# henrycharlesworth/settlers_of_catan_RL

Hardware: AMD Instinct MI355X
Metric: Catan env-steps/sec at 65k parallel games (higher is better)
Workload: dtype u8/u32 (integer bitboards); 1 GPU; configs[1]: 65 536 parallel envs per GPU, random policy, step+mask only, bit-exact vs CPU oracle; games_per_gpu=65536, games_total=65536, validate_actions=True, auto_reset=True, parallelism=games sharded over 1 GPU(s), no collective

## Files before the change

### settlers_of_catan_rl_amd/csrc/catan_kernels.hip

```cpp
#include <hip/hip_runtime.h>
#include <stdint.h>

#include "catan_state.h"

#define CATAN_TABLE static __device__ __constant__ const
#define CATAN_FN static __device__ __forceinline__
#define CATAN_TOPOLOGY_CODE
#include "catan_topology.inc"

namespace catan {

#define DEVI __device__ __forceinline__

constexpr int BLOCK = 256;
constexpr u64 ALL54 = (1ull << 54) - 1;

constexpr int MT_RING = 8192, MT_AHEAD = 6144, MT_AHEAD_PY = 1024;
struct MtGen { u32 mt[624]; u32 idx; u32 produced; u32 ring[MT_RING]; };
struct MtPair { MtGen np, py; u32 cons_py; };
struct BoardCfg {
    int32_t randomise;
    int32_t fixed_terrain;
    int32_t fixed_numbers;
    int8_t terrain[19];
// ... 1409 lines not shown
            tmask &= tmask - 1;
            const int r0 = (s.b(B_TILE + t) & 15) - 1;
            const u64 tm = tct[t];
            u32 add = 0;
#pragma unroll
            for (int p = 0; p < 4; p++) add |= (u32)(__popcll(st[p] & tm) + 2 * __popcll(ct[p] & tm)) << (8 * p);
#pragma unroll
            for (int k = 0; k < 5; k++) alloc[k] += (k == r0) ? add : 0u;
        }
    }
    const int res_order[5] = { R_WOOD, R_ORE, R_BRICK, R_WHEAT, R_SHEEP };
    u32 okbits = 0;
#pragma unroll
    for (int i = 0; i < 5; i++) {
        int r0 = res_order[i];
        u32 al = alloc[r0];
        int tot = (al & 255) + ((al >> 8) & 255) + ((al >> 16) & 255) + (al >> 24);
        int bank = s.b(B_BANK + r0);
        if (tot <= bank) { okbits |= 1u << r0; if (tot) s.sb(B_BANK + r0, bank - tot); }
    }
    if (tk) { const long long t1 = clock_fenced(); tk[1] = (u32)(t1 - t0); t0 = t1; }
    u32 mw = 0;
#pragma unroll
    for (int r = 0; r < 4; r++) mw |= ((okbits >> r) & 1) ? 0xFFu << (8 * r) : 0u;
    const u32 mc = ((okbits >> 4) & 1) ? 0xFFFFu : 0u;
    u32 pw[4], tw[4], pc[4], tc[4];
#pragma unroll
    for (int X = 0; X < 4; X++) {
        int hand[5], tot = 0;
#pragma unroll
        for (int r = 0; r < 5; r++) { hand[r] = s.res(X, r); tot += hand[r]; }
        int add[5], bound[5];
#pragma unroll
        for (int r = 0; r < 5; r++) add[r] = ((okbits >> r) & 1) ? (int)((alloc[r] >> (8 * X)) & 255) : 0;
#pragma unroll
        for (int i = 0; i < 5; i++) { const int r = res_order[i]; tot += add[r]; bound[r] = tot; }
#pragma unroll
        for (int r = 0; r < 5; r++) s.spb(X, P_RES + r, hand[r] + add[r]);
        pw[X] = (u32)add[0] | ((u32)add[1] << 8) | ((u32)add[2] << 16) | ((u32)add[3] << 24);
        tw[X] = (u32)bound[0] | ((u32)bound[1] << 8) | ((u32)bound[2] << 16) | ((u32)bound[3] << 24);
        pc[X] = (u32)add[4] * 0x0101u; tc[X] = (u32)bound[4] * 0x0101u;
    }
    int base[12];
    u32 ea[12], eb[12], ec[12], guard = 0;
#pragma unroll
    for (int X = 0; X < 4; X++)
#pragma unroll
        for (int j = 0; j < 3; j++) {
            const int o = j + (j >= X ? 1 : 0), k = X * 3 + j;
            base[k] = W_EST + (o * 3 + label_of(seatof, o, X)) * 3;
            ea[k] = s.w(base[k]); eb[k] = s.w(base[k] + 1); ec[k] = s.w(base[k] + 2);
            guard |= ea[k] | eb[k] | ec[k] | (ea[k] + pw[X]) | (eb[k] + pw[X]) | (ec[k] + pc[X]) | pw[X] | pc[X] | tw[X] | tc[X];
        }
    if ((guard & H4) == 0) {
#pragma unroll
        for (int X = 0; X < 4; X++)
#pragma unroll
            for (int j = 0; j < 3; j++) {
                const int k = X * 3 + j;
                s.sw(base[k], swar_addmin(ea[k], pw[X], tw[X], mw));
                s.sw(base[k] + 1, swar_addmin(eb[k], pw[X], tw[X], mw));
                s.sw(base[k] + 2, swar_addmin(ec[k], pc[X], tc[X], mc));
            }
    } else {
        for (int X = 0; X < 4; X++)
            for (int o = 0; o < 4; o++)
                if (o != X) est_apply(s, o, label_of(seatof, o, X), pw[X], 0u, tw[X], mw, pc[X], 0u, tc[X], mc);
    }
    if (tk) tk[2] = (u32)(clock_fenced() - t0);
    return roll;
}

template <class S>
DEVI void update_largest_army(const S& s) {
    const int order[4] = { 1, 0, 3, 2 };
    int max_count = 0, who = -1;
#pragma unroll
    for (int i = 0; i < 4; i++) {
        int p = order[i], k = s.pb(p, P_ARMY);
        if (k >= 3 && k > max_count) { max_count = k; who = p; }
    }
    if (who < 0) return;
    int la = s.b(B_LA_PLAYER);
    if (la == 0) { s.sb(B_LA_PLAYER, who + 1); s.sb(B_LA_COUNT, max_count); s.spb(who, P_VP, s.pb(who, P_VP) + 2); }
    else if (la == who + 1) s.sb(B_LA_COUNT, max_count);
    else if (max_count > s.b(B_LA_COUNT)) {
        s.spb(la - 1, P_VP, s.pb(la - 1, P_VP) - 2);
        s.sb(B_LA_PLAYER, who + 1); s.sb(B_LA_COUNT, max_count);
        s.spb(who, P_VP, s.pb(who, P_VP) + 2);
    }
}

struct StepCfg { int validate; int dense_reward; double win_reward; double annealing; Limits lim; int auto_reset;
                 double* reward64;
                 unsigned long long* prof;
                 u32* prof_wave;
                 int prof_timeline;
                 int bin_order; };
constexpr int LRF_PROF_ROW = 4128, LRF_PROF_ROWS = 2000;
constexpr int LRH_PROF_ROW = 6128, LRH_PROF_ROWS = 1000;
constexpr long prof_wave_rows(long N) { return (N / 16 + 17 > LRH_PROF_ROW + LRH_PROF_ROWS) ? N / 16 + 17 : LRH_PROF_ROW + LRH_PROF_ROWS; }
constexpr int PROF_PHASES = 8;
constexpr int PROF_TOTAL = 2 * PROF_PHASES + 4;
constexpr int PROF_WORDS = PROF_TOTAL + 42;
DEVI void prof_mark(const StepCfg& cfg, int phase, long long& t_prev) {
    if (cfg.prof_wave != nullptr) {
        const long long t = wall_clock64();
        if ((threadIdx.x & 63) == 0 && !(cfg.prof_timeline && phase == 2))
            cfg.prof_wave[((long)blockIdx.x * (blockDim.x >> 6) + (threadIdx.x >> 6)) * 8 + phase] = (u32)(t - t_prev);
        t_prev = wall_clock64();
        return;
    }
    if (cfg.prof == nullptr) return;
    long long t = wall_clock64();
    if ((threadIdx.x & 63) == 0) {
        unsigned long long dt = (unsigned long long)(t - t_prev);
        atomicAdd(&cfg.prof[phase], dt);
        atomicMax(&cfg.prof[PROF_PHASES + phase], dt);
    }
    t_prev = wall_clock64();
}

struct Pending { u32* ctr; u64* req[3]; u64* heavy[2]; u64* heavy2; u8* type; u8* who; u64* len; u32* arrive; i32* resets[2][3]; u8* busy;
                 u64* spec;
                 i32* lists;
                 int bsel;
                 int bclear;
                 int fa, ftag, sa, stag;
                 int sample;
                 int lrq_clear;
                 int bnext;
                 int brel;
                 u32* bctr;
                 int nsub;
               };
constexpr int CTR_WORDS = 96;
constexpr int BIN_SETS = 4;
DEVI int lrq_ctr(int fl) { return fl < 2 ? 4 + fl : 7; }
constexpr int NBINS = 18, BIN_NOOP = NBINS - 1;
static_assert(16 + BIN_SETS * NBINS <= CTR_WORDS, "the sets of bin counts live in ctr[16 ..]");
constexpr int BCTR_PAD = 32;
constexpr int MAX_SUBS = 16;
DEVI u32* sub_ctr(const Pending& pend, int set, int bin, int sub) { return pend.bctr + (((long)set * NBINS + bin) * pend.nsub + sub) * BCTR_PAD; }
DEVI i32* sub_list(const Pending& pend, int set, int bin, int sub, long N) { return pend.lists + (((long)set * NBINS + bin) * pend.nsub + sub) * N; }
DEVI int bin_of(int t, int card) {
    if (t < 0 || t > 12) return BIN_NOOP;
    if (t != T_PLAYDEV) return t;
    card = min(max(card, 0), 4);
    return card >= 1 ? 12 + card : t;
}
__device__ constexpr int BIN_ORDER_LPT[18] = { 0, 9, 7, 11, 16, 2, 14, 3, 5, 4, 13, 1, 12, 8, 15, 6, 10, 17 };
DEVI int type_of_bin(int bin) { return bin <= 12 ? bin : (bin < BIN_NOOP ? T_PLAYDEV : -1); }

template <class S>
DEVI void sample_enqueue_lane(const Ctx& c, const S& s, const u32 (&m)[MASK_WORDS], const Pending& pend, u32* __restrict__ mpk) {
    const long e = s.e;
    u32* row = mpk + e * MPK_STRIDE;
    int a[ACTION_WORDS];
    const int t = sample_random(c, s, m, row[ROW_CTR], a, (u32*)nullptr, (u8*)nullptr, 0, 0);
    uint4* dst = reinterpret_cast<uint4*>(row + ROW_ACT);
#pragma unroll
    for (int i = 0; i < 4; i++) dst[i] = make_uint4((u32)a[4 * i], (u32)a[4 * i + 1], (u32)a[4 * i + 2], (u32)a[4 * i + 3]);
    *reinterpret_cast<uint2*>(row + ROW_ACT + 16) = make_uint2((u32)a[16], (u32)a[17]);
    if (pend.brel >= 0) {
        const int bin = bin_of(t, a[4]), sub = (int)(e & (pend.nsub - 1));
        const u32 rank = atomicAdd(sub_ctr(pend, pend.brel, bin, sub), 1u);
        sub_list(pend, pend.brel, bin, sub, c.N)[rank] = (i32)e;
    } else {
        const u32 rank = atomicAdd(&pend.ctr[11 + 4 * pend.sa], 1u);
        pend.resets[pend.sa][2][rank] = (i32)e;
    }
}

struct StepCfg;
DEVI void prof_mark(const StepCfg& cfg, int phase, long long& t_prev);
struct StepScratch { LrWave lr; };

template <int LR, class S>
DEVI void finish_step(const Ctx& c, const S& s, StepScratch* scratch, const StepCfg& cfg, int lane, bool doit, int type,
                      int lr_who, int len, float* __restrict__ reward, u8* __restrict__ done, u32* __restrict__ mpk,
                      long long& tprof, u32 nbr_c, u32 nbr_e, const Pending& pend, int rlist, bool clear_busy,
                      u32* m_out = nullptr, bool* m_valid = nullptr, LrCache* lc = nullptr) {
    const long e = s.e;
    if constexpr (LR != 0) {
        bool cut = false;
        int holder = 0, hcount = 0;
        if constexpr (LR == 2) prof_mark(cfg, 2, tprof);
        if (doit && lr_who >= 0) {
            s.spb(lr_who, P_CURLP, len);
            holder = s.b(B_LR_PLAYER); hcount = s.b(B_LR_COUNT);
            if (holder == 0) {
                if (len >= 5) { s.sb(B_LR_PLAYER, lr_who + 1); s.sb(B_LR_COUNT, len); s.spb(lr_who, P_VP, s.pb(lr_who, P_VP) + 2); }
            } else if (holder == lr_who + 1) {
                if (hcount > len) cut = true; else s.sb(B_LR_COUNT, len);
            } else if (len > hcount) {
                s.spb(holder - 1, P_VP, s.pb(holder - 1, P_VP) - 2);
                s.spb(lr_who, P_VP, s.pb(lr_who, P_VP) + 2);
                s.sb(B_LR_PLAYER, lr_who + 1); s.sb(B_LR_COUNT, len);
            }
        }
        if constexpr (LR == 2) prof_mark(cfg, 5, tprof);
        if constexpr (LR == 2) {
        if (__ballot(cut)) {
            int max_len = len, player = lr_who;
            bool tied = false;
            for (int o = 0; o < 4; o++) {
                const bool mine = cut && o != lr_who;
                const bool need = mine && !lc->valid(o);
                const u64 found = coop_longest_path_packed(need, s, o, scratch->lr, 0, nbr_c, nbr_e);
                if (need) lc->set(o, found & LR_VMASK);
                if (mine) {
                    const int pl = lr_len(lc->get(o));
                    if (pl == max_len) tied = true;
                    else if (pl > max_len) { max_len = pl; tied = false; player = o; }
                }
            }
            if (cut) {
                if (max_len >= 5) {
                    if (tied) {
                        if (player == lr_who) s.sb(B_LR_COUNT, len);
                        else { s.sb(B_LR_PLAYER, 0); s.sb(B_LR_COUNT, 0); s.spb(lr_who, P_VP, s.pb(lr_who, P_VP) - 2); }
                    } else {
                        s.sb(B_LR_PLAYER, player + 1); s.sb(B_LR_COUNT, max_len);
                        s.spb(player, P_VP, s.pb(player, P_VP) + 2);
                        s.spb(lr_who, P_VP, s.pb(lr_who, P_VP) - 2);
                    }
                } else { s.sb(B_LR_PLAYER, 0); s.sb(B_LR_COUNT, 0); s.spb(lr_who, P_VP, s.pb(lr_who, P_VP) - 2); }
            }
        }
        }
    }
    if constexpr (LR == 2) prof_mark(cfg, 3, tprof);
    bool want_reset = false;
    if (doit) {
        const int dict_order[4] = { 1, 3, 2, 0 };
        int vps[4];
#pragma unroll
        for (int p = 0; p < 4; p++) vps[p] = s.pb(p, P_VP);
        int winner = 0;
#pragma unroll
        for (int i = 0; i < 4; i++) if (vps[dict_order[i]] >= 10) winner = dict_order[i] + 1;
        bool dn = winner != 0 && type >= 0;
        double rw[4];
#pragma unroll
        for (int p = 0; p < 4; p++) {
            double r = 0.0;
            if (type >= 0) {
                if (cfg.dense_reward) {
                    r += (double)(5 * (vps[p] - s.b(B_CURVP + p)));
                    if (type == T_PLAYDEV) r += 5.0;
                    if (type == T_ROBBER) r += 1.0;
                    if (type == T_DISCARD) r -= 0.3;
                    if (type == T_CITY) r += 2.5;
                    r *= cfg.annealing;
                }
                s.sb(B_CURVP + p, vps[p]);
                if (dn && winner == p + 1) r += cfg.win_reward;
            }
            rw[p] = r;
        }
        *reinterpret_cast<float4*>(reward + s.e * 4) = make_float4((float)rw[0], (float)rw[1], (float)rw[2], (float)rw[3]);
        if (cfg.reward64) {
            *reinterpret_cast<double2*>(cfg.reward64 + s.e * 4) = make_double2(rw[0], rw[1]);
            *reinterpret_cast<double2*>(cfg.reward64 + s.e * 4 + 2) = make_double2(rw[2], rw[3]);
        }
        if (dn) s.sb(B_WINNER, winner);
        done[s.e] = dn ? 1 : 0;
        want_reset = dn && cfg.auto_reset;
        if (want_reset) pend.resets[pend.sa][rlist][atomicAdd(&pend.ctr[9 + 4 * pend.sa + rlist], 1u)] = (i32)s.e;
        if (want_reset) pend.busy[s.e] = (u8)pend.stag;
        else if (lr_who >= 0 && clear_busy) pend.busy[s.e] = 0;
    }
    if constexpr (LR == 2) prof_mark(cfg, 4, tprof);
    if (doit && !want_reset) {
        u32 m[MASK_WORDS];
        compute_masks(s, m, cfg.lim);
        if (m_out != nullptr) {
#pragma unroll
            for (int i = 0; i < MASK_WORDS; i++) m_out[i] = m[i];
            *m_valid = true;
        } else {
#pragma unroll
            for (int i = 0; i < MASK_WORDS; i++) mpk[e * MPK_STRIDE + i] = m[i];
        }
    }
    prof_mark(cfg, 6, tprof);
}

template <int G, bool SAMPLE = false>
__global__ __launch_bounds__(64) void k_step(Ctx c, const i32* __restrict__ actions, u32* __restrict__ mpk,
                                             float* __restrict__ reward, u8* __restrict__ done,
                                             u32* __restrict__ err, StepCfg cfg, Pending pend, const u32* __restrict__ bins) {
    constexpr int TSG = G + 1;
    typedef StLT<TSG> StG;
    __shared__ u32 tile_all[1][ROWS_HOT * TSG];
    __shared__ u64 tct_all[1][20];
    const int lane = threadIdx.x & 63, wib = threadIdx.x >> 6;
    const int wv = (int)blockIdx.x + wib;
    u32* const tile = tile_all[wib];
    u64* const tct = tct_all[wib];
    if constexpr (SAMPLE) {
        if (wv == 0)
            for (int i = lane; i < NBINS * pend.nsub; i += 64) pend.bctr[((long)pend.bclear * NBINS * pend.nsub + i) * BCTR_PAD] = 0;
        if (wv == 0 && lane == 0 && pend.lrq_clear >= 0) pend.ctr[lrq_ctr(pend.lrq_clear)] = 0;
    } else if (wv == 0 && lane < NBINS) pend.ctr[16 + NBINS * pend.bclear + lane] = 0;
    int bin = -1, cnt = 0, first = 0;
    u32 subc[SAMPLE ? MAX_SUBS : 1];
    if constexpr (SAMPLE) {
        u32 mine[MAX_SUBS], tot = 0;
#pragma unroll
        for (int j = 0; j < MAX_SUBS; j++) mine[j] = (lane < NBINS && j < pend.nsub) ? *sub_ctr(pend, pend.bsel, lane, j) : 0u;
#pragma unroll
        for (int j = 0; j < MAX_SUBS; j++) tot += mine[j];
        const int pos = wv * G;
        int start = 0;
#pragma unroll
        for (int kk = 0; kk < NBINS; kk++) {
            const int k = cfg.bin_order ? BIN_ORDER_LPT[kk] : kk;
            const int ck = __builtin_amdgcn_readlane((int)tot, k), len = (ck + G - 1) & ~(G - 1);
            if (bin < 0 && pos < start + len) { bin = k; cnt = ck; first = pos - start; }
            start += len;
        }
        if (bin < 0) return;
#pragma unroll
        for (int j = 0; j < MAX_SUBS; j++) subc[j] = (u32)__builtin_amdgcn_readlane((int)mine[j], bin);
    } else {
        const int pos = wv * G;
        int start = 0;
#pragma unroll
        for (int kk = 0; kk < NBINS; kk++) {
            const int k = cfg.bin_order ? BIN_ORDER_LPT[kk] : kk;
            const int ck = (int)bins[k], len = (ck + G - 1) & ~(G - 1);
            if (bin < 0 && pos < start + len) { bin = k; cnt = ck; first = pos - start; }
            start += len;
        }
        if (bin < 0) return;
    }
    const int rnk = first + lane;
    long e = 0x7fffffffL;
    if (lane < G && rnk < cnt) {
        if constexpr (SAMPLE) {
            int sub = 0;
            u32 off = (u32)rnk;
#pragma unroll
            for (int j = 0; j < MAX_SUBS - 1; j++) if (sub == j && j + 1 < pend.nsub && off >= subc[j]) { off -= subc[j]; sub = j + 1; }
            e = (long)sub_list(pend, pend.bsel, bin, sub, c.N)[off];
        } else e = (long)pend.lists[((long)pend.bsel * NBINS + bin) * c.N + rnk];
    }
    long long tprof = (cfg.prof || cfg.prof_wave) ? wall_clock64() : 0;
    if (cfg.prof_wave != nullptr && cfg.prof_timeline && lane == 0) cfg.prof_wave[(long)wv * 8 + 2] = (u32)tprof;
    const bool live = e < c.n;
    int type = live ? type_of_bin(bin) : -1;
    if (live && type < 0) {
        *reinterpret_cast<float4*>(reward + e * 4) = make_float4(0.f, 0.f, 0.f, 0.f);
        if (cfg.reward64) { double2* r64 = reinterpret_cast<double2*>(cfg.reward64 + e * 4); r64[0] = make_double2(0.0, 0.0); r64[1] = make_double2(0.0, 0.0); }
        done[e] = 0;
    }
    if (__ballot(type >= 0) == 0) return;
    if (__ballot(type == T_ROLL) != 0 && lane < 19) tct[lane] = topo_tile_corners(lane);
    u32 nbr_c, nbr_e;
    lr_load_nbr(lane, nbr_c, nbr_e);
    int a[ACTION_WORDS];
    const bool t_board = type == T_SETTLE || type == T_ROAD || type == T_CITY;
    const bool t_est = t_board || type == T_BUYDEV || bin == 12 + C_YOP || bin == 12 + C_MONO || type == T_EXCHANGE || type == T_RESPOND ||
                       type == T_ROLL || type == T_STEAL || type == T_DISCARD;
    const bool w_board = __ballot(type >= 0 && t_board) != 0, w_est = __ballot(type >= 0 && t_est) != 0;
    u32 dctr = 0;
    if (w_est) stage_in_all<true, G, SAMPLE>(tile, c.R, actions, type >= 0 ? (int)e : -1, lane, a, mpk, &dctr);
    else stage_in_all<false, G, SAMPLE>(tile, c.R, actions, type >= 0 ? (int)e : -1, lane, a, mpk, &dctr);
    __builtin_amdgcn_wave_barrier();
    StG s(tile + (lane < G ? lane : G - 1), c.R, c.N, e);
    prof_mark(cfg, 0, tprof);
    bool rejected = false;
    if (cfg.validate && type >= 0 && !action_valid(s, a)) { atomicAdd(err, 1u); type = -1; rejected = true; }
    if (rejected) {
        *reinterpret_cast<float4*>(reward + e * 4) = make_float4(0.f, 0.f, 0.f, 0.f);
        if (cfg.reward64) { double2* r64 = reinterpret_cast<double2*>(cfg.reward64 + e * 4); r64[0] = make_double2(0.0, 0.0); r64[1] = make_double2(0.0, 0.0); }
        done[e] = 0;
    }
    a[1] = min(max(a[1], 0), 53); a[2] = min(max(a[2], 0), 72); a[3] = min(max(a[3], 0), 18);
    a[4] = min(max(a[4], 0), 4); a[6] = min(max(a[6], 0), 2);
    a[15] = min(max(a[15], 0), 4); a[16] = min(max(a[16], 0), 4); a[17] = min(max(a[17], 0), 4);

#ifdef CATAN_FINE_PROF
    prof_mark(cfg, 4, tprof);
#endif
    const int order = s.b(B_ORDER), seatof = s.b(B_SEATOF);
    const int pid = s.b(B_GO);
    int flags = s.flags();
    int lr_who = -1, lr_edge = 127, lr_len_now = 0;
    bool lr_inline = false;
    const long long t_sw0 = cfg.prof_wave ? clock_fenced() : 0;

    switch (type) {
    case T_SETTLE: {
        int cn = a[1];
        if (!(flags & F_INITIAL)) { pay(s, pid, R_WHEAT, 1); pay(s, pid, R_SHEEP, 1); pay(s, pid, R_WOOD, 1); pay(s, pid, R_BRICK, 1); }
        s.set_settle(pid, s.settle(pid) | (1ull << cn));
        int slot = CORNER_HSLOT[cn];
        if (slot != 255) {
            int hid = s.b(B_HARB + slot);
            int bitpos = hid == 0 ? R_ORE + 1 : hid == 1 ? R_SHEEP + 1 : hid == 2 ? R_WHEAT + 1 : hid == 3 ? R_WOOD + 1 : hid == 4 ? R_BRICK + 1 : 0;
            s.spb(pid, P_HARB, s.pb(pid, P_HARB) | (1 << bitpos));
        }
        s.spb(pid, P_SLEFT, s.pb(pid, P_SLEFT) - 1);
        s.spb(pid, P_VP, s.pb(pid, P_VP) + 1);
        LrCache lc;
        lc.load(s.P);
        if (lc.settle_invalidate(pid, cn)) lc.store(s.P);
        if (flags & F_INITIAL) {
            int k = s.pb(pid, P_ISET) + 1;
            s.spb(pid, P_ISET, k);
            if (k == 2) {
                D5 d = d5_zero();
                int touched = 0;
                for (int q = 0; q < 3; q++) {
                    int t = CORNER_TILE[cn][q];
                    if (t == 255) continue;
                    int r0 = (s.b(B_TILE + t) & 15) - 1;
                    if (r0 < 0) continue;
                    s.spb(pid, P_RES + r0, s.pb(pid, P_RES + r0) + 1);
                    s.spb(pid, P_VIS + r0, s.pb(pid, P_VIS + r0) + 1);
                    s.sb(B_BANK + r0, s.b(B_BANK + r0) - 1);
                    d5_add(d, r0, 1); touched |= 1 << r0;
                }
                update_estimates(s, seatof, d, touched, pid, -1);
                s.spb(pid, P_ISECOND, cn);
            }
        } else {
            D5 d; d.v[R_BRICK] = -1; d.v[R_WOOD] = -1; d.v[R_ORE] = 0; d.v[R_SHEEP] = -1; d.v[R_WHEAT] = -1;
            update_estimates(s, seatof, d, 0b11011, pid, -1);
            int lrp = s.b(B_LR_PLAYER);
            if (lrp) {
                lr_who = lrp - 1;
                if (lc.valid(lr_who) && lr_len(lc.get(lr_who)) >= s.b(B_LR_COUNT)) { lr_inline = true; lr_len_now = lr_len(lc.get(lr_who)); }
            }
        }
// ... 147 lines not shown
                lost |= (u32)k << (8 * o); got += k;
            }
            s.spb(pid, P_RES + r0, s.pb(pid, P_RES + r0) + got);
            s.spb(pid, P_VIS + r0, s.pb(pid, P_VIS + r0) + got);
            update_estimates_monopoly(s, seatof, pid, r0, lost);
        } else if (card == C_YOP) {
            for (int i = 0; i < 2; i++) {
                int r0 = i == 0 ? a[15] : a[16];
                int bank = s.b(B_BANK + r0);
                if (bank > 0) {
                    s.sb(B_BANK + r0, bank - 1);
                    s.spb(pid, P_RES + r0, s.pb(pid, P_RES + r0) + 1);
                    s.spb(pid, P_VIS + r0, s.pb(pid, P_VIS + r0) + 1);
                    update_estimates1(s, seatof, r0, 1, pid);
                }
            }
        }
        s.sb(B_FLAGS, flags);
        break;
    }
    case T_BUYDEV: {
        pay(s, pid, R_SHEEP, 1); pay(s, pid, R_ORE, 1); pay(s, pid, R_WHEAT, 1);
        D5 d = d5_zero(); d.v[R_SHEEP] = -1; d.v[R_ORE] = -1; d.v[R_WHEAT] = -1;
        update_estimates(s, seatof, d, (1 << R_SHEEP) | (1 << R_ORE) | (1 << R_WHEAT), pid, -1);
        int pl = s.b(B_PILE_LEN) - 1;
        int card = s.pile(pl);
        s.sb(B_PILE_LEN, pl);
        int nh = s.pb(pid, P_NHID);
        s.set_hidden(pid, nh, card);
        s.spb(pid, P_NHID, nh + 1);
        s.spb(pid, P_HCNT + card, s.pb(pid, P_HCNT + card) + 1);
        s.sb(B_BOUGHT + card, s.b(B_BOUGHT + card) + 1);
        break;
    }
    case T_EXCHANGE: {
        int give = a[15], want = a[16];
        int hb = s.pb(pid, P_HARB);
        int rate = ((hb >> (give + 1)) & 1) ? 2 : ((hb & 1) ? 3 : 4);
        s.spb(pid, P_RES + want, s.pb(pid, P_RES + want) + 1);
        s.spb(pid, P_VIS + want, s.pb(pid, P_VIS + want) + 1);
        s.spb(pid, P_RES + give, s.pb(pid, P_RES + give) - rate);
        s.spb(pid, P_VIS + give, max(s.pb(pid, P_VIS + give) - rate, 0));
        s.sb(B_BANK + give, s.b(B_BANK + give) + rate);
        s.sb(B_BANK + want, s.b(B_BANK + want) - 1);
        D5 d = d5_zero();
        d5_add(d, want, 1); d5_add(d, give, -rate);
        update_estimates(s, seatof, d, (1 << want) | (1 << give), pid, -1);
        break;
    }
    case T_PROPOSE: {
        flags |= F_MUST_RESPOND;
        s.sb(B_FLAGS, flags);
        s.sb(B_TRADE_PROP, pid);
        s.sb(B_TRADE_TGT, player_at_label(order, seatof, pid, a[6]));
        int ng = 0, nr = 0;
        bool stop = false;
        for (int i = 0; i < 4; i++) { int v = a[7 + i]; if (v <= 0 || v > 5) stop = true; s.sb(B_TRADE_GIVE + i, stop ? 0 : v); if (!stop) ng++; }
        stop = false;
        for (int i = 0; i < 4; i++) { int v = a[11 + i]; if (v <= 0 || v > 5) stop = true; s.sb(B_TRADE_RECV + i, stop ? 0 : v); if (!stop) nr++; }
        s.sb(B_TRADE_NG, ng); s.sb(B_TRADE_NR, nr);
        s.sb(B_TRADES, min(s.b(B_TRADES) + 1, 255));
        break;
    }
    case T_RESPOND: {
        if (a[5] == 0) {
            int p1 = s.b(B_TRADE_PROP), p2 = s.b(B_TRADE_TGT);
            int ng = s.b(B_TRADE_NG), nr = s.b(B_TRADE_NR);
            int g[5] = { 0, 0, 0, 0, 0 }, rc[5] = { 0, 0, 0, 0, 0 };
            for (int i = 0; i < 4; i++) if (i < ng) {
                const int r0 = s.b(B_TRADE_GIVE + i) - 1;
#pragma unroll
                for (int k = 0; k < 5; k++) g[k] += (k == r0) ? 1 : 0;
            }
            for (int i = 0; i < 4; i++) if (i < nr) {
                const int r0 = s.b(B_TRADE_RECV + i) - 1;
#pragma unroll
                for (int k = 0; k < 5; k++) rc[k] += (k == r0) ? 1 : 0;
            }
            D5 d1, d2;
            int t1 = 0;
            int r1[5], v1[5], r2[5], v2[5];
#pragma unroll
            for (int k = 0; k < 5; k++) { r1[k] = s.pb(p1, P_RES + k); v1[k] = s.pb(p1, P_VIS + k); r2[k] = s.pb(p2, P_RES + k); v2[k] = s.pb(p2, P_VIS + k); }
#pragma unroll
            for (int k = 0; k < 5; k++) {
                s.spb(p1, P_RES + k, r1[k] - g[k] + rc[k]);
                s.spb(p1, P_VIS + k, max(v1[k] - g[k], 0) + rc[k]);
                s.spb(p2, P_RES + k, r2[k] + g[k] - rc[k]);
                s.spb(p2, P_VIS + k, max(v2[k] + g[k] - rc[k], 0));
                d1.v[k] = rc[k] - g[k]; d2.v[k] = g[k] - rc[k];
                t1 |= (g[k] | rc[k]) ? 1 << k : 0;
            }
            update_estimates(s, seatof, d1, t1, p1, -1);
            update_estimates(s, seatof, d2, t1, p2, -1);
        }
        flags &= ~F_MUST_RESPOND;
        s.sb(B_FLAGS, flags);
        s.sb(B_TRADE_PROP, 0); s.sb(B_TRADE_TGT, 0); s.sb(B_TRADE_NG, 0); s.sb(B_TRADE_NR, 0);
        for (int i = 0; i < 4; i++) { s.sb(B_TRADE_GIVE + i, 0); s.sb(B_TRADE_RECV + i, 0); }
        break;
    }
    case T_DISCARD: {
        int who = s.b(B_DISC), r0 = a[17];
        s.spb(who, P_RES + r0, s.pb(who, P_RES + r0) - 1);
        s.sb(B_BANK + r0, s.b(B_BANK + r0) + 1);
        update_estimates1(s, seatof, r0, -1, who);
        if (s.total(who) <= 7) {
            int n = s.b(B_NDISC);
            for (int i = 0; i + 1 < 4; i++) s.sb(B_DISC + i, (i + 1 < n) ? s.b(B_DISC + i + 1) : 0);
            s.sb(B_DISC + 3, 0);
            s.sb(B_NDISC, n - 1);
        }
        break;
    }
    default: break;
    }
    if (cfg.prof_wave != nullptr) {
        const long long t_sw1 = clock_fenced();
        if (lane == 0) cfg.prof_wave[(long)wv * 8 + 3] = ((u32)(t_sw0 - tprof) & 0xFFFFu) | ((u32)(t_sw1 - t_sw0) << 16);
    }
    if (type >= 0 && type != T_RESPOND && type != T_ENDTURN && type != T_DISCARD) s.sw(W_ACTIONS, s.w(W_ACTIONS) + 1);

    if (cfg.prof_wave != nullptr && lane == 0) cfg.prof_wave[(long)wv * 8 + 5] = (u32)(type >= 0 ? bin + 1 : 0);
    if (cfg.prof != nullptr && cfg.prof_wave == nullptr && lane == 0) {
        const int t0 = live ? actions[e * ACTION_WORDS] : 13;
        const int tb = (t0 < 0 || t0 > 12) ? 13 : t0;
        const unsigned long long dt = (unsigned long long)(wall_clock64() - tprof);
        atomicAdd(&cfg.prof[PROF_TOTAL + tb], dt); atomicAdd(&cfg.prof[PROF_TOTAL + 14 + tb], 1ull);
        atomicMax(&cfg.prof[PROF_TOTAL + 28 + tb], dt);
    }
    prof_mark(cfg, 1, tprof);
    const int len = lr_len_now;
    const bool pending = lr_who >= 0 && !lr_inline;
    if (pending) {
        const u32 slot = atomicAdd(&pend.ctr[lrq_ctr(pend.fa)], 1u);
        pend.req[pend.fa][slot] = (u64)e | ((u64)lr_edge << 40) | ((u64)lr_who << 56);
        if (pend.stag < 2) {
            bool may_end = false;
            if (type == T_ROAD) {
                may_end = s.pb(lr_who, P_VP) >= 8 && s.b(B_LR_PLAYER) != lr_who + 1;
            } else {
#pragma unroll
                for (int p = 0; p < 4; p++) may_end |= s.pb(p, P_VP) >= 8;
            }
            if (may_end) pend.spec[atomicAdd(&pend.ctr[6], 1u)] = (u64)e;
        }
        pend.type[e] = (u8)(type + 1);
        pend.who[e] = (u8)lr_who;
        pend.busy[e] = (u8)pend.ftag;
    }
    prof_mark(cfg, 2, tprof);
    u32 m_new[MASK_WORDS];
    bool have_masks = false;
    finish_step<1>(c, s, (StepScratch*)nullptr, cfg, lane, type >= 0 && !pending, type, lr_inline ? lr_who : -1, len, reward, done, mpk, tprof, nbr_c, nbr_e,
                   pend, 0, false, m_new, &have_masks);
    int an[ACTION_WORDS] = { 0, 0, 0, 0, 0, 0, 0, 0, 0, 0, 0, 0, 0, 0, 0, 0, 0, 0 };
    u32 abase = 0, arank = 0;
    int aleader = 0, anb = -1;
    if constexpr (SAMPLE) {
        const long long t_s0 = cfg.prof_wave ? clock_fenced() : 0;
        if (type >= 0) dctr++;
        int nb = -1;
        if (have_masks) nb = bin_of(sample_random(c, s, m_new, dctr, an, (u32*)nullptr, (u8*)nullptr, 0, 0), an[4]);
        else if (type >= 0) mpk[e * MPK_STRIDE + ROW_CTR] = dctr;
        const long long t_s1 = cfg.prof_wave ? clock_fenced() : 0;
        u32 rank = 0, cntb = 0;
        int leader = 0;
#pragma unroll
        for (int b = 0; b < NBINS - 1; b++) {
            const u64 mk = __ballot(nb == b);
            if (nb == b) { rank = (u32)__popcll(mk & ((1ull << lane) - 1)); cntb = (u32)__popcll(mk); leader = __ffsll((long long)mk) - 1; }
        }
        if (nb >= 0 && lane == leader) abase = atomicAdd(sub_ctr(pend, pend.bnext, nb, wv & (pend.nsub - 1)), cntb);
        arank = rank; aleader = leader; anb = nb;
        if (cfg.prof_wave != nullptr) {
            const long long t_s2 = clock_fenced();
            if (lane == 0) cfg.prof_wave[(long)wv * 8 + 4] = ((u32)(t_s1 - t_s0) & 0xFFFFu) | ((u32)(t_s2 - t_s1) << 16);
        }
    }
    __builtin_amdgcn_wave_barrier();
    if (w_board) stage_out<28, 0, G>(tile, c.R, (type >= 0 || rejected) ? (int)e : -1, lane);
    else if (w_est) stage_out<21, 7, G>(tile, c.R, (type >= 0 || rejected) ? (int)e : -1, lane);
    else stage_out<12, 16, G>(tile, c.R, (type >= 0 || rejected) ? (int)e : -1, lane);
    __builtin_amdgcn_wave_barrier();
    if constexpr (SAMPLE) {
        abase = __shfl(abase, aleader);
        if (anb >= 0) sub_list(pend, pend.bnext, anb, wv & (pend.nsub - 1), c.N)[abase + arank] = (i32)e;
    }
    if constexpr (SAMPLE) stage_out_row<G>(tile, mpk, have_masks ? (int)e : -1, lane, m_new, an, dctr);
    else stage_out_masks<G>(tile, mpk, have_masks ? (int)e : -1, lane, m_new);
    prof_mark(cfg, 7, tprof);
    if (cfg.prof_wave != nullptr && cfg.prof_timeline) {
        u32 hw, xcc;
        asm volatile("s_getreg_b32 %0, hwreg(HW_REG_HW_ID)" : "=s"(hw));
        asm volatile("s_getreg_b32 %0, hwreg(HW_REG_XCC_ID)" : "=s"(xcc));
        if (lane == 0) cfg.prof_wave[(long)wv * 8 + 3] = (hw & 0x0FFFFFFFu) | ((xcc & 15u) << 28);
    }
}

constexpr u64 LR_GAME_MASK = (1ull << 40) - 1;
struct LrPlan { bool through; int u, v; };
DEVI LrPlan lr_plan(const LrCache& lc, int who, int edge) {
    LrPlan pl;
    pl.through = edge < 72 && lc.valid(who);
    const int ed = edge < 72 ? edge : 0;
    pl.u = EDGE_CORNER[ed][0]; pl.v = EDGE_CORNER[ed][1];
    return pl;
}
DEVI int lr_apply(LrCache& lc, int who, bool through, u64 found) {
    const u64 old = lc.get(who);
    const int flen = (int)(found >> 54);
    if (through && lr_len(old) >= flen) return lr_len(old);
    lc.set(who, found & LR_VMASK);
    return flen;
}
constexpr int CTR_HEAVY2 = 88;
constexpr int LRF_TIER1 = 0, LRF_SPLIT = 1, LRF_MID = 2;
template <int MODE>
__global__ __launch_bounds__(64) void k_lr_finish(Ctx c, u32* __restrict__ mpk, float* __restrict__ reward, u8* __restrict__ done,
                                                  StepCfg cfg, Pending pend, int fl, int budget, unsigned long long* stat,
                                                  unsigned long long* slow_ctr) {
    __shared__ StepScratch scratch;
    __shared__ __attribute__((aligned(16))) u32 rec[ROWS_HOT];
    const int lane = threadIdx.x;
    u32 nbr_c, nbr_e;
    lr_load_nbr(lane, nbr_c, nbr_e);
    constexpr bool SPLIT = MODE == LRF_SPLIT, MID = MODE == LRF_MID;
    const u32 count = MID ? pend.ctr[8 + 4 * pend.sa] : pend.ctr[lrq_ctr(fl)];
    if (!MID && blockIdx.x == 0 && lane == 0 && slow_ctr != nullptr) { atomicAdd(&slow_ctr[0], (unsigned long long)count); atomicAdd(&slow_ctr[2], 1ull); }
    StepCfg cfg2 = cfg;
    cfg2.prof = nullptr;
    cfg2.prof_wave = cfg.prof_wave != nullptr && blockIdx.x < LRF_PROF_ROWS && count <= gridDim.x && c.N >= 65536 ? cfg.prof_wave + LRF_PROF_ROW * 8 : nullptr;
    for (u32 r = blockIdx.x; r < count; r += gridDim.x) {
        long long tprof = wall_clock64();
        const u64 rq = MID ? pend.heavy[pend.sa][r] : pend.req[fl][r];
        const long e = (long)(rq & LR_GAME_MASK);
        const int who = (int)(rq >> 56), edge = (int)((rq >> 40) & 127);
        __builtin_amdgcn_wave_barrier();
        if (lane < ROWS_HOT / 4) reinterpret_cast<uint4*>(rec)[lane] = reinterpret_cast<const uint4*>(c.R + e * REC)[lane];
        __builtin_amdgcn_wave_barrier();
        prof_mark(cfg2, 0, tprof);
        StL1 s(rec, c.R, c.N, e);
        LrCache lc;
        lc.load(s.P);
        const LrPlan pl = lr_plan(lc, who, edge);
        u64 BL = 0;
        for (int o = 0; o < 4; o++) if (o != who) BL |= s.settle(o) | s.city(o);
        const u64 found = lr_wave_search(s.road_lo(who), s.road_hi(who), BL, pl.through, pl.u, pl.v, scratch.lr, budget, nbr_c, nbr_e, stat);
        if (MID && found == LR_OVERFLOW) {
            if (lane == 0) pend.heavy2[atomicAdd(&pend.ctr[CTR_HEAVY2], 1u)] = rq;
            continue;
        }
        if (found == LR_OVERFLOW) {
            if (lane == 0) {
                const u32 slot = atomicAdd(&pend.ctr[8 + 4 * pend.sa], 1u);
                pend.heavy[pend.sa][slot] = rq; pend.len[e] = 0; pend.arrive[e] = 0; pend.busy[e] = (u8)pend.stag;
                if (slow_ctr != nullptr) atomicAdd(&slow_ctr[1], 1ull);
            }
            continue;
        }
        const int len = lr_apply(lc, who, pl.through, found);
        prof_mark(cfg2, 1, tprof);
        if constexpr (SPLIT) {
            if (!(s.b(B_LR_PLAYER) == who + 1 && s.b(B_LR_COUNT) > len)) {
                if (lane == 0) { lc.store(s.P); pend.len[e] = (1ull << 63) | (u64)len; }
                continue;
            }
            if (lane == 0) pend.len[e] = 0;
        }
        u32 mn[MASK_WORDS];
        bool mv = false;
        finish_step<2>(c, s, &scratch, cfg2, lane, lane == 0, (int)pend.type[e] - 1, who, len, reward, done, mpk, tprof, nbr_c, nbr_e, pend,
                       MID ? 1 : (pend.stag < 2 ? 2 : 0), MID ? pend.stag < 2 : pend.ftag < 2, pend.sample ? mn : nullptr, pend.sample ? &mv : nullptr, &lc);
        if (mv) {
#pragma unroll
            for (int i = 0; i < MASK_WORDS; i++) mpk[e * MPK_STRIDE + i] = mn[i];
            sample_enqueue_lane(c, s, mn, pend, mpk);
        }
        __builtin_amdgcn_wave_barrier();
        if (lane < ROWS_HOT / 4) reinterpret_cast<uint4*>(c.R + e * REC)[lane] = reinterpret_cast<const uint4*>(rec)[lane];
        if (lane == 0) lc.store(s.P);
        prof_mark(cfg2, 7, tprof);
    }
}

__global__ __launch_bounds__(64) void k_lr_complete(Ctx c, u32* __restrict__ mpk, float* __restrict__ reward, u8* __restrict__ done,
                                                    StepCfg cfg, Pending pend, int fl) {
    __shared__ u32 tile[ROWS_HOT * TS];
    const int lane = threadIdx.x;
    const u32 count = pend.ctr[lrq_ctr(fl)];
    cfg.prof = nullptr; cfg.prof_wave = nullptr;
    for (u32 base = blockIdx.x * 64u; base < count; base += gridDim.x * 64u) {
        const u32 r = base + lane;
        long e = -1;
        int who = 0, len = 0, type = -1;
        if (r < count) {
            const u64 rq = pend.req[fl][r];
            const long g = (long)(rq & LR_GAME_MASK);
            const u64 L = pend.len[g];
            if (L >> 63) { e = g; who = (int)(rq >> 56); len = (int)(L & 0xFFu); type = (int)pend.type[g] - 1; pend.len[g] = 0; }
        }
        if (__ballot(e >= 0) == 0) continue;
        __builtin_amdgcn_wave_barrier();
        stage_in(tile, c.R, (int)e, lane);
        __builtin_amdgcn_wave_barrier();
        StL s(tile + lane, c.R, c.N, e >= 0 ? e : 0);
        u32 m_new[MASK_WORDS];
        bool have_masks = false;
        long long tprof = 0;
        finish_step<1>(c, s, (StepScratch*)nullptr, cfg, lane, e >= 0, type, who, len, reward, done, mpk, tprof, 0u, 0u, pend,
                       pend.stag < 2 ? 2 : 0, pend.ftag < 2, m_new, &have_masks);
        int an[ACTION_WORDS] = { 0, 0, 0, 0, 0, 0, 0, 0, 0, 0, 0, 0, 0, 0, 0, 0, 0, 0 };
        u32 dctr = 0;
        if (pend.sample && have_masks) {
            dctr = mpk[e * MPK_STRIDE + ROW_CTR];
            const int nb = bin_of(sample_random(c, s, m_new, dctr, an, (u32*)nullptr, (u8*)nullptr, 0, 0), an[4]), sub = (int)(e & (pend.nsub - 1));
            sub_list(pend, pend.brel, nb, sub, c.N)[atomicAdd(sub_ctr(pend, pend.brel, nb, sub), 1u)] = (i32)e;
        }
        __builtin_amdgcn_wave_barrier();
        stage_out<28, 0, 64>(tile, c.R, (int)e, lane);
        __builtin_amdgcn_wave_barrier();
        if (pend.sample) stage_out_row<64>(tile, mpk, have_masks ? (int)e : -1, lane, m_new, an, dctr);
        else stage_out_masks<64>(tile, mpk, have_masks ? (int)e : -1, lane, m_new);
    }
}

__global__ __launch_bounds__(LR_HEAVY_THREADS) void k_lr_heavy(Ctx c, const u32* __restrict__ req_count,
                                                              const u64* __restrict__ req, u64* __restrict__ out64, int round_iters,
                                                              u32* __restrict__ mpk, float* __restrict__ reward, u8* __restrict__ done,
                                                              StepCfg cfg, Pending pend) {
    __shared__ u64 adj[54];
    __shared__ u64 pool_seen[LR_POOL];
    __shared__ unsigned short pool_cd[LR_POOL];
    __shared__ unsigned long long best_all;
    __shared__ u64 blk_all;
    __shared__ int pool_n, is_last;
    __shared__ __attribute__((aligned(16))) lrstk_t path[54][LR_HEAVY_THREADS];
    static_assert(sizeof(StepScratch) + ROWS_HOT * 4 + 64 <= sizeof(lrstk_t) * 54 * LR_HEAVY_THREADS, "the completion reuses the DFS stacks");
    const int tid = threadIdx.x;
    const u32 nreq = *req_count;
    const u32 LR_SPLIT = nreq * 8 <= gridDim.x ? 8u : (nreq * 4 <= gridDim.x ? 4u : (nreq * 2 <= gridDim.x ? 2u : 1u));
    const u32 count = nreq * LR_SPLIT;
    u32 nbr_c, nbr_e;
    lr_load_nbr(tid < 54 ? tid : 0, nbr_c, nbr_e);
    StepCfg cfg2 = cfg;
    cfg2.prof = nullptr; cfg2.prof_wave = nullptr;
    u32* const hp = cfg.prof_wave != nullptr && blockIdx.x < LRH_PROF_ROWS && c.N >= 65536 ? cfg.prof_wave + (LRH_PROF_ROW + blockIdx.x) * 8 : nullptr;
    for (u32 r = blockIdx.x; r < count; r += gridDim.x) {
        const long long hp_t0 = wall_clock64();
        u32 hp_rounds = 0;
        const u64 rq = req[r / LR_SPLIT];
        const int part = (int)(r % LR_SPLIT);
        const long game = (long)(rq & LR_GAME_MASK);
        const int pid = (int)(rq >> 56), edge = (int)((rq >> 40) & 127);
        St s(c.R, c.N, game);
        LrCache lc;
        lc.load(s.P);
        const LrPlan pl = lr_plan(lc, pid, edge);
        __syncthreads();
        if (tid < 54) {
            u64 BL = 0;
            for (int o = 0; o < 4; o++) if (o != pid) BL |= s.settle(o) | s.city(o);
            adj[tid] = lr_adj_of(tid, nbr_c, nbr_e, s.road_lo(pid), s.road_hi(pid), BL);
            if (tid == 0) blk_all = BL;
        }
        if (tid == 0) { pool_n = 0; best_all = 0ull; }
        __syncthreads();
        const LrGraph G{ adj, blk_all, pl.v };
        Dfs t;
        if (pl.through) {
            const bool wide = LR_SPLIT >= 4;
            dfs_seed_through(t, wide ? part < 4 : part == 0, pl.u, pl.v, adj[pl.u]);
            dfs_walk_prefix<true>(t, G, wide ? part * LR_HEAVY_THREADS + tid : tid, wide ? 6 : 5);
        } else {
            const int st = tid % 54, code = tid / 54;
            dfs_seed_full(t, st, adj[st]);
            t.active = t.active && code < 16 && ((u32)st % LR_SPLIT) == (u32)part;
            dfs_walk_prefix<true>(t, G, code, 2);
        }
        const DfsQueue q{ pool_seen, pool_cd, &pool_n, LR_POOL };
        bool hint = true;
        const long long hp_t1 = wall_clock64();
        while (true) {
            hp_rounds++;
            for (int it = 0; it < round_iters; it++) dfs_iter<true>(t, G, &path[0][tid], LR_HEAVY_THREADS, hint, q);
            __syncthreads();
            if (!t.active) {
                const int qi = atomicSub(&pool_n, 1) - 1;
                if (qi >= 0) dfs_take(t, G, pool_seen[qi], pool_cd[qi]);
                else atomicAdd(&pool_n, 1);
            }
            const int busy = __syncthreads_count(t.active);
            if (busy == 0) break;
            hint = busy < LR_HEAVY_THREADS;
        }
        const long long hp_t2 = wall_clock64();
        if (t.best > 0) atomicMax(&best_all, (unsigned long long)lr_pack(t.best, t.bseen));
        __syncthreads();
        if (tid == 0) {
            if (best_all > 0) atomicMax(reinterpret_cast<unsigned long long*>(&out64[game]), best_all);
            __threadfence();
            is_last = atomicAdd(&pend.arrive[game], 1u) == LR_SPLIT - 1 ? 1 : 0;
        }
        __syncthreads();
        const long long hp_t3 = wall_clock64();
        if (is_last && tid < 64) {
            StepScratch* scratch = reinterpret_cast<StepScratch*>(&path[0][0]);
            u32* rec = reinterpret_cast<u32*>(reinterpret_cast<char*>(&path[0][0]) + ((sizeof(StepScratch) + 63) & ~size_t(63)));
            const int lane = tid;
            const u64 found = atomicMax(reinterpret_cast<unsigned long long*>(&out64[game]), 0ull);
            if (lane < ROWS_HOT / 4) reinterpret_cast<uint4*>(rec)[lane] = reinterpret_cast<const uint4*>(c.R + game * REC)[lane];
            __builtin_amdgcn_wave_barrier();
            StL1 sl(rec, c.R, c.N, game);
            u32 nc, ne;
            lr_load_nbr(lane, nc, ne);
            const int len = lr_apply(lc, pid, pl.through, found);
            long long tprof = 0;
            u32 mn[MASK_WORDS];
            bool mv = false;
            finish_step<2>(c, sl, scratch, cfg2, lane, lane == 0, (int)pend.type[game] - 1, pid, len, reward, done, mpk, tprof, nc, ne, pend,
                           1, pend.stag < 2, pend.sample ? mn : nullptr, pend.sample ? &mv : nullptr, &lc);
            if (mv) {
#pragma unroll
                for (int i = 0; i < MASK_WORDS; i++) mpk[game * MPK_STRIDE + i] = mn[i];
                sample_enqueue_lane(c, sl, mn, pend, mpk);
            }
            __builtin_amdgcn_wave_barrier();
            if (lane < ROWS_HOT / 4) reinterpret_cast<uint4*>(c.R + game * REC)[lane] = reinterpret_cast<const uint4*>(rec)[lane];
            if (lane == 0) lc.store(sl.P);
        }
        if (hp != nullptr && tid == 0 && r == blockIdx.x) {
            const long long hp_t4 = wall_clock64();
            hp[0] = (u32)(hp_t1 - hp_t0); hp[1] = hp_rounds; hp[2] = (u32)(hp_t2 - hp_t1); hp[3] = (u32)(hp_t3 - hp_t2);
            hp[4] = is_last ? (u32)(hp_t4 - hp_t3) : 0u; hp[5] = LR_SPLIT | ((pl.through ? 1u : 0u) << 8) | ((u32)part << 16);
            hp[6] = (u32)hp_t0; hp[7] = (u32)hp_t4;
        }
    }
}

__global__ __launch_bounds__(BLOCK) void k_release_tags(Ctx c, u8* __restrict__ busy) {
    const long e = (long)blockIdx.x * BLOCK + threadIdx.x;
    if (e < c.N && busy[e] >= 2) busy[e] = 0;
}

__global__ __launch_bounds__(BLOCK) void k_sample_first(Ctx c, u32* __restrict__ mpk, const u32* __restrict__ pctr, Pending pend, int set) {
    __shared__ u32 hist[NBINS], base[NBINS];
    if (threadIdx.x < NBINS) hist[threadIdx.x] = 0;
    __syncthreads();
    St s(c.R, c.N, (long)blockIdx.x * BLOCK + threadIdx.x);
    int bin = BIN_NOOP;
    if (s.e < c.n) {
        u32* row = mpk + s.e * MPK_STRIDE;
        u32 m[MASK_WORDS];
#pragma unroll
        for (int i = 0; i < MASK_WORDS; i++) m[i] = row[i];
        int a[ACTION_WORDS];
        const u32 d = pctr[s.e];
        bin = bin_of(sample_random(c, s, m, d, a, (u32*)nullptr, (u8*)nullptr, 0, 0), a[4]);
        uint4* dst = reinterpret_cast<uint4*>(row + ROW_ACT);
#pragma unroll
        for (int i = 0; i < 4; i++) dst[i] = make_uint4((u32)a[4 * i], (u32)a[4 * i + 1], (u32)a[4 * i + 2], (u32)a[4 * i + 3]);
        dst[4] = make_uint4((u32)a[16], (u32)a[17], d, 0u);
    }
    u32 rank = 0;
    const bool valid = s.e < c.n;
    if (valid) rank = atomicAdd(&hist[bin], 1u);
    __syncthreads();
    const int sub = (int)(blockIdx.x & (pend.nsub - 1));
    if (threadIdx.x < NBINS) base[threadIdx.x] = hist[threadIdx.x] ? atomicAdd(sub_ctr(pend, set, threadIdx.x, sub), hist[threadIdx.x]) : 0u;
    __syncthreads();
    if (valid) sub_list(pend, set, bin, sub, c.N)[base[bin] + rank] = (i32)s.e;
}
__global__ __launch_bounds__(BLOCK) void k_release_window(Ctx c, const u32* __restrict__ mpk, const u32* __restrict__ count_p, const i32* __restrict__ list,
                                                         Pending pend, int set) {
    const u32 count = *count_p;
    for (u32 r = blockIdx.x * BLOCK + threadIdx.x; r < count; r += gridDim.x * BLOCK) {
        const long e = list[r];
        const u32* row = mpk + e * MPK_STRIDE;
        const int bin = bin_of((int)row[ROW_ACT], (int)row[ROW_ACT + 4]), sub = (int)(e & (pend.nsub - 1));
        sub_list(pend, set, bin, sub, c.N)[atomicAdd(sub_ctr(pend, set, bin, sub), 1u)] = (i32)e;
    }
}
__global__ __launch_bounds__(BLOCK) void k_finish_rollout(Ctx c, const u32* __restrict__ mpk, u32* __restrict__ pctr, u8* __restrict__ busy) {
    const long e = (long)blockIdx.x * BLOCK + threadIdx.x;
    if (e < c.n) pctr[e] = mpk[e * MPK_STRIDE + ROW_CTR];
    if (e < c.N) busy[e] = 0;
}

DEVI void wave_reset_game(const Ctx& c, long e, u32* rec, ResetScratch& sc, int lane, u32* __restrict__ mpk, Limits lim, u8* busy,
                           unsigned long long* prof = nullptr, u32* __restrict__ dstR = nullptr, const Pending* pend = nullptr, bool board_only = false) {
    u32* const outR = dstR ? dstR : c.R;
    __builtin_amdgcn_wave_barrier();
    if (lane < ROWS_HOT / 4) reinterpret_cast<uint4*>(rec)[lane] = reinterpret_cast<const uint4*>(c.R + e * REC)[lane];
    __builtin_amdgcn_wave_barrier();
    StL1 s(rec, outR, c.N, e);
    Rng mine = rng_load(c, s);
    const u32 blk0 = mine.draws >> 2;
#pragma unroll
    for (int b = 0; b < RND_WORDS / 256; b++) {
        u32 o[4];
        mine.block(blk0 + b * 64 + lane, o);
        const int at = (b * 64 + lane) * 4;
        sc.rnd[at] = o[0]; sc.rnd[at + 1] = o[1]; sc.rnd[at + 2] = o[2]; sc.rnd[at + 3] = o[3];
    }
    for (int r = ROWS_HOT + lane; r < REC; r += 64) outR[e * REC + r] = 0;
    __builtin_amdgcn_wave_barrier();
    RngBuf rb;
    rb.buf = sc.rnd; rb.base = blk0 * 4; rb.avail = RND_WORDS; rb.slow = mine;
    const long long t0 = prof ? wall_clock64() : 0;
    const BoardCfg* bc = c.bcfg != nullptr ? c.bcfg + c.bcfg_idx[e] : nullptr;
    if (lane == 0) reset_part1(s, rb, sc, ROWS_HOT, bc);
    __builtin_amdgcn_wave_barrier();
    const bool tokens_done = tokens_fixed(bc) || reset_tokens_parallel(sc, lane);
    __builtin_amdgcn_wave_barrier();
    if (lane == 0) {
        reset_part2(s, rb, sc, tokens_done, board_only);
        if (prof) {
            const unsigned long long dt = (unsigned long long)(wall_clock64() - t0);
            atomicAdd(&prof[5], dt); atomicMax(&prof[PROF_PHASES + 5], dt);
            atomicAdd(&prof[3], (unsigned long long)(rb.slow.draws - mine.draws)); atomicMax(&prof[PROF_PHASES + 3], (unsigned long long)(rb.slow.draws - mine.draws));
            atomicAdd(&prof[4], 1ull);
        }
        if (mpk != nullptr) {
            u32 m[MASK_WORDS];
            compute_masks(s, m, lim);
#pragma unroll
            for (int i = 0; i < MASK_WORDS; i++) mpk[e * MPK_STRIDE + i] = m[i];
            if (pend != nullptr && pend->sample) sample_enqueue_lane(c, s, m, *pend, mpk);
        }
    }
    __builtin_amdgcn_wave_barrier();
    if (lane < ROWS_HOT / 4) reinterpret_cast<uint4*>(outR + e * REC)[lane] = reinterpret_cast<const uint4*>(rec)[lane];
    if (lane == 0 && busy != nullptr) busy[e] = 0;
}
__global__ __launch_bounds__(64) void k_reset_list(Ctx c, u32* __restrict__ mpk, Limits lim, const u32* __restrict__ count_p,
                                                   const i32* __restrict__ list, u8* __restrict__ busy, unsigned long long* prof,
                                                   const u32* __restrict__ spec_count_p, const u64* __restrict__ spec_list,
                                                   u32* __restrict__ specR, u32* __restrict__ spec_mpk, u32 epoch, Pending pend) {
    __shared__ __attribute__((aligned(16))) u32 rec[ROWS_HOT];
    __shared__ ResetScratch sc;
    const u32 count = *count_p, scount = spec_list ? *spec_count_p : 0u;
    for (u32 r = blockIdx.x; r < count + scount; r += gridDim.x) {
        if (r < count) wave_reset_game(c, list[r], rec, sc, threadIdx.x, mpk, lim, busy, prof, nullptr, &pend);
        else {
            const long e = (long)(spec_list[r - count] & 0x00FFFFFFFFFFFFFFull);
            wave_reset_game(c, e, rec, sc, threadIdx.x, spec_mpk, lim, nullptr, nullptr, specR);
            if (threadIdx.x == 0) spec_mpk[e * MPK_STRIDE + MPK_STRIDE - 1] = epoch;
        }
    }
}
__global__ __launch_bounds__(64) void k_install_list(Ctx c, u32* __restrict__ mpk, Limits lim, const u32* __restrict__ count_p,
                                                     const i32* __restrict__ list, u8* __restrict__ busy, const u32* __restrict__ specR,
                                                     const u32* __restrict__ spec_mpk, u32 epoch, u32* __restrict__ err) {
    __shared__ __attribute__((aligned(16))) u32 rec[ROWS_HOT];
    __shared__ ResetScratch sc;
    const u32 count = *count_p;
    const int lane = threadIdx.x;
    for (u32 r = blockIdx.x; r < count; r += gridDim.x) {
        const long e = list[r];
        if (spec_mpk[e * MPK_STRIDE + MPK_STRIDE - 1] != epoch) {
            if (lane == 0) atomicAdd(err + 2, 1u);
            wave_reset_game(c, e, rec, sc, lane, mpk, lim, busy, nullptr);
            continue;
        }
        if (lane < REC / 4) reinterpret_cast<uint4*>(c.R + e * REC)[lane] = reinterpret_cast<const uint4*>(specR + e * REC)[lane];
        if (lane < 3)
            reinterpret_cast<uint4*>(mpk + e * MPK_STRIDE)[lane] = reinterpret_cast<const uint4*>(spec_mpk + e * MPK_STRIDE)[lane];
        if (lane == 0 && busy != nullptr) busy[e] = 0;
    }
}
__global__ __launch_bounds__(64) void k_reset(Ctx c, const u8* __restrict__ sel, int board_only) {
    __shared__ __attribute__((aligned(16))) u32 rec[ROWS_HOT];
    __shared__ ResetScratch sc;
    for (long e = blockIdx.x; e < c.N; e += gridDim.x) {
        if (sel != nullptr && (e >= c.n || sel[e] == 0)) continue;
        wave_reset_game(c, e, rec, sc, threadIdx.x, nullptr, Limits{ -1, -1 }, nullptr, nullptr, nullptr, nullptr, board_only != 0);
    }
}
__global__ __launch_bounds__(BLOCK) void k_board_cfg_index(long n, long N, const u8* __restrict__ src, int n_cfgs, u8* __restrict__ dst,
// ... 450 lines not shown
```

Baseline: 1.052 billion env-steps/s.

## Compute masks and sample once in k_step; deferred completions enqueue from stored row

```diff
diff --git a/settlers_of_catan_rl_amd/csrc/catan_kernels.hip b/settlers_of_catan_rl_amd/csrc/catan_kernels.hip
--- a/settlers_of_catan_rl_amd/csrc/catan_kernels.hip
+++ b/settlers_of_catan_rl_amd/csrc/catan_kernels.hip
@@ -1585,6 +1585,20 @@
 __device__ constexpr int BIN_ORDER_LPT[18] = { 0, 9, 7, 11, 16, 2, 14, 3, 5, 4, 13, 1, 12, 8, 15, 6, 10, 17 };
 DEVI int type_of_bin(int bin) { return bin <= 12 ? bin : (bin < BIN_NOOP ? T_PLAYDEV : -1); }
 
+DEVI void enqueue_lane(const Ctx& c, long e, int t, int card, const Pending& pend) {
+    if (pend.brel >= 0) {
+        const int bin = bin_of(t, card), sub = (int)(e & (pend.nsub - 1));
+        const u32 rank = atomicAdd(sub_ctr(pend, pend.brel, bin, sub), 1u);
+        sub_list(pend, pend.brel, bin, sub, c.N)[rank] = (i32)e;
+    } else {
+        const u32 rank = atomicAdd(&pend.ctr[11 + 4 * pend.sa], 1u);
+        pend.resets[pend.sa][2][rank] = (i32)e;
+    }
+}
+DEVI void enqueue_from_row(const Ctx& c, long e, const Pending& pend, const u32* __restrict__ mpk) {
+    const u32* row = mpk + e * MPK_STRIDE;
+    enqueue_lane(c, e, (int)row[ROW_ACT], (int)row[ROW_ACT + 4], pend);
+}
 template <class S>
 DEVI void sample_enqueue_lane(const Ctx& c, const S& s, const u32 (&m)[MASK_WORDS], const Pending& pend, u32* __restrict__ mpk) {
     const long e = s.e;
@@ -1595,14 +1609,7 @@
 #pragma unroll
     for (int i = 0; i < 4; i++) dst[i] = make_uint4((u32)a[4 * i], (u32)a[4 * i + 1], (u32)a[4 * i + 2], (u32)a[4 * i + 3]);
     *reinterpret_cast<uint2*>(row + ROW_ACT + 16) = make_uint2((u32)a[16], (u32)a[17]);
-    if (pend.brel >= 0) {
-        const int bin = bin_of(t, a[4]), sub = (int)(e & (pend.nsub - 1));
-        const u32 rank = atomicAdd(sub_ctr(pend, pend.brel, bin, sub), 1u);
-        sub_list(pend, pend.brel, bin, sub, c.N)[rank] = (i32)e;
-    } else {
-        const u32 rank = atomicAdd(&pend.ctr[11 + 4 * pend.sa], 1u);
-        pend.resets[pend.sa][2][rank] = (i32)e;
-    }
+    enqueue_lane(c, e, t, a[4], pend);
 }
 
 struct StepCfg;
@@ -1610,11 +1617,10 @@
 struct StepScratch { LrWave lr; };
 
 template <int LR, class S>
-DEVI void finish_step(const Ctx& c, const S& s, StepScratch* scratch, const StepCfg& cfg, int lane, bool doit, int type,
-                      int lr_who, int len, float* __restrict__ reward, u8* __restrict__ done, u32* __restrict__ mpk,
+DEVI void finish_step(const Ctx& c, const S& s, StepScratch* scratch, const StepCfg& cfg, int lane, bool doit, bool masks, int type,
+                      int lr_who, int len, float* __restrict__ reward, u8* __restrict__ done,
                       long long& tprof, u32 nbr_c, u32 nbr_e, const Pending& pend, int rlist, bool clear_busy,
-                      u32* m_out = nullptr, bool* m_valid = nullptr, LrCache* lc = nullptr) {
-    const long e = s.e;
+                      u32* m_out, bool* goes_on, LrCache* lc = nullptr) {
     if constexpr (LR != 0) {
         bool cut = false;
         int holder = 0, hcount = 0;
@@ -1705,17 +1711,12 @@
         else if (lr_who >= 0 && clear_busy) pend.busy[s.e] = 0;
     }
     if constexpr (LR == 2) prof_mark(cfg, 4, tprof);
-    if (doit && !want_reset) {
+    if ((doit || masks) && !want_reset) *goes_on = true;
+    if (masks && !want_reset) {
         u32 m[MASK_WORDS];
         compute_masks(s, m, cfg.lim);
-        if (m_out != nullptr) {
-#pragma unroll
-            for (int i = 0; i < MASK_WORDS; i++) m_out[i] = m[i];
-            *m_valid = true;
-        } else {
-#pragma unroll
-            for (int i = 0; i < MASK_WORDS; i++) mpk[e * MPK_STRIDE + i] = m[i];
-        }
+#pragma unroll
+        for (int i = 0; i < MASK_WORDS; i++) m_out[i] = m[i];
     }
     prof_mark(cfg, 6, tprof);
 }
@@ -2169,7 +2170,7 @@
     prof_mark(cfg, 2, tprof);
     u32 m_new[MASK_WORDS];
     bool have_masks = false;
-    finish_step<1>(c, s, (StepScratch*)nullptr, cfg, lane, type >= 0 && !pending, type, lr_inline ? lr_who : -1, len, reward, done, mpk, tprof, nbr_c, nbr_e,
+    finish_step<1>(c, s, (StepScratch*)nullptr, cfg, lane, type >= 0 && !pending, type >= 0, type, lr_inline ? lr_who : -1, len, reward, done, tprof, nbr_c, nbr_e,
                    pend, 0, false, m_new, &have_masks);
     int an[ACTION_WORDS] = { 0, 0, 0, 0, 0, 0, 0, 0, 0, 0, 0, 0, 0, 0, 0, 0, 0, 0 };
     u32 abase = 0, arank = 0;
@@ -2178,8 +2179,10 @@
         const long long t_s0 = cfg.prof_wave ? clock_fenced() : 0;
         if (type >= 0) dctr++;
         int nb = -1;
-        if (have_masks) nb = bin_of(sample_random(c, s, m_new, dctr, an, (u32*)nullptr, (u8*)nullptr, 0, 0), an[4]);
-        else if (type >= 0) mpk[e * MPK_STRIDE + ROW_CTR] = dctr;
+        if (have_masks) {
+            const int tn = sample_random(c, s, m_new, dctr, an, (u32*)nullptr, (u8*)nullptr, 0, 0);
+            if (!pending) nb = bin_of(tn, an[4]);
+        } else if (type >= 0) mpk[e * MPK_STRIDE + ROW_CTR] = dctr;
         const long long t_s1 = cfg.prof_wave ? clock_fenced() : 0;
         u32 rank = 0, cntb = 0;
         int leader = 0;
@@ -2285,15 +2288,10 @@
             }
             if (lane == 0) pend.len[e] = 0;
         }
-        u32 mn[MASK_WORDS];
-        bool mv = false;
-        finish_step<2>(c, s, &scratch, cfg2, lane, lane == 0, (int)pend.type[e] - 1, who, len, reward, done, mpk, tprof, nbr_c, nbr_e, pend,
-                       MID ? 1 : (pend.stag < 2 ? 2 : 0), MID ? pend.stag < 2 : pend.ftag < 2, pend.sample ? mn : nullptr, pend.sample ? &mv : nullptr, &lc);
-        if (mv) {
-#pragma unroll
-            for (int i = 0; i < MASK_WORDS; i++) mpk[e * MPK_STRIDE + i] = mn[i];
-            sample_enqueue_lane(c, s, mn, pend, mpk);
-        }
+        bool goes_on = false;
+        finish_step<2>(c, s, &scratch, cfg2, lane, lane == 0, false, (int)pend.type[e] - 1, who, len, reward, done, tprof, nbr_c, nbr_e, pend,
+                       MID ? 1 : (pend.stag < 2 ? 2 : 0), MID ? pend.stag < 2 : pend.ftag < 2, nullptr, &goes_on, &lc);
+        if (goes_on && pend.sample) enqueue_from_row(c, e, pend, mpk);
         __builtin_amdgcn_wave_barrier();
         if (lane < ROWS_HOT / 4) reinterpret_cast<uint4*>(c.R + e * REC)[lane] = reinterpret_cast<const uint4*>(rec)[lane];
         if (lane == 0) lc.store(s.P);
@@ -2322,23 +2320,13 @@
         stage_in(tile, c.R, (int)e, lane);
         __builtin_amdgcn_wave_barrier();
         StL s(tile + lane, c.R, c.N, e >= 0 ? e : 0);
-        u32 m_new[MASK_WORDS];
-        bool have_masks = false;
+        bool goes_on = false;
         long long tprof = 0;
-        finish_step<1>(c, s, (StepScratch*)nullptr, cfg, lane, e >= 0, type, who, len, reward, done, mpk, tprof, 0u, 0u, pend,
-                       pend.stag < 2 ? 2 : 0, pend.ftag < 2, m_new, &have_masks);
-        int an[ACTION_WORDS] = { 0, 0, 0, 0, 0, 0, 0, 0, 0, 0, 0, 0, 0, 0, 0, 0, 0, 0 };
-        u32 dctr = 0;
-        if (pend.sample && have_masks) {
-            dctr = mpk[e * MPK_STRIDE + ROW_CTR];
-            const int nb = bin_of(sample_random(c, s, m_new, dctr, an, (u32*)nullptr, (u8*)nullptr, 0, 0), an[4]), sub = (int)(e & (pend.nsub - 1));
-            sub_list(pend, pend.brel, nb, sub, c.N)[atomicAdd(sub_ctr(pend, pend.brel, nb, sub), 1u)] = (i32)e;
-        }
+        finish_step<1>(c, s, (StepScratch*)nullptr, cfg, lane, e >= 0, false, type, who, len, reward, done, tprof, 0u, 0u, pend,
+                       pend.stag < 2 ? 2 : 0, pend.ftag < 2, nullptr, &goes_on);
+        if (goes_on && pend.sample) enqueue_from_row(c, e, pend, mpk);
         __builtin_amdgcn_wave_barrier();
         stage_out<28, 0, 64>(tile, c.R, (int)e, lane);
-        __builtin_amdgcn_wave_barrier();
-        if (pend.sample) stage_out_row<64>(tile, mpk, have_masks ? (int)e : -1, lane, m_new, an, dctr);
-        else stage_out_masks<64>(tile, mpk, have_masks ? (int)e : -1, lane, m_new);
     }
 }
 
@@ -2433,15 +2421,10 @@
             lr_load_nbr(lane, nc, ne);
             const int len = lr_apply(lc, pid, pl.through, found);
             long long tprof = 0;
-            u32 mn[MASK_WORDS];
-            bool mv = false;
-            finish_step<2>(c, sl, scratch, cfg2, lane, lane == 0, (int)pend.type[game] - 1, pid, len, reward, done, mpk, tprof, nc, ne, pend,
-                           1, pend.stag < 2, pend.sample ? mn : nullptr, pend.sample ? &mv : nullptr, &lc);
-            if (mv) {
-#pragma unroll
-                for (int i = 0; i < MASK_WORDS; i++) mpk[game * MPK_STRIDE + i] = mn[i];
-                sample_enqueue_lane(c, sl, mn, pend, mpk);
-            }
+            bool goes_on = false;
+            finish_step<2>(c, sl, scratch, cfg2, lane, lane == 0, false, (int)pend.type[game] - 1, pid, len, reward, done, tprof, nc, ne, pend,
+                           1, pend.stag < 2, nullptr, &goes_on, &lc);
+            if (goes_on && pend.sample) enqueue_from_row(c, game, pend, mpk);
             __builtin_amdgcn_wave_barrier();
             if (lane < ROWS_HOT / 4) reinterpret_cast<uint4*>(c.R + game * REC)[lane] = reinterpret_cast<const uint4*>(rec)[lane];
             if (lane == 0) lc.store(sl.P);
```

Measured after the change: 1.061 billion env-steps/s (median of 6 runs). No clear change (+0.9%).
